# EricLBuehler/mistral.rs

Measured on AMD Instinct MI355X. Metric: decode_tokens_per_sec, higher is better.
Workload: dtype q4_k/q6_k weights x q8_k activations (int8 dot, f32 accumulate: the reference CPU path's arithmetic); 1 GPU; Llama-3-8B GGUF Q4_K_M, TP=1, 512 prefill / 1599 decode, batch 1, paged KV bf16 (block 32); parallelism=tp1

## Files before the change

### include/mrs_hip_ext.h

```cpp
#ifndef MRS_HIP_EXT_H
#define MRS_HIP_EXT_H
#include <stddef.h>
#include <stdint.h>
#ifdef __cplusplus
extern "C" {
#endif

int mrs_decode_gemv_supported(int ggml_type);
int mrs_decode_qkv(const void *wq, const void *wk, const void *wv, int tq, int tk, int tv, int nq, int nk, int nv, int K,
                   const float *h, const float *norm_w, float eps, float *q_out, void *k_cache, void *v_cache,
                   const int64_t *slot_mapping, const int32_t *positions, const float *cos_t, const float *sin_t,
                   int head_dim, int rot_pairs, int num_kv_heads, int block_size, int b, void *stream);
int mrs_decode_gate_up(const void *wg, const void *wu, int type, int n, int K, const float *h, const float *norm_w, float eps,
                       int activation, void *y_out, int y_out_stride, int b, void *stream);
int mrs_decode_proj(const void *w, int type, int n, int K, const void *y_q8_1, int stride_col_y, float *out, int out_stride,
                    int accumulate, int b, void *stream);
int mrs_decode_proj_scaled(const void *w, int type, int n, int K, const void *y_q8_1, int stride_col_y, float *out, int out_stride,
                           float resid_scale, int b, void *stream);
int mrs_vec_add_f32(float *a, const float *b, size_t n, void *stream);
int mrs_decode_norm_proj(const void *w, int type, int n, int K, const float *h, const float *norm_w, float eps, float *out,
                         int out_stride, int b, void *stream);
typedef struct { const void *planes; int type; long long n, k; } mrs_dec_mat;
int mrs_dec_supported(int ggml_type);
size_t mrs_dec_repack_bytes(int ggml_type, long long n, long long k);
int mrs_dec_repack(const void *gguf_blocks, int ggml_type, long long n, long long k, void *planes, void *stream);
int mrs_dec_qkv(const mrs_dec_mat *wq, const mrs_dec_mat *wk, const mrs_dec_mat *wv, const float *h, int ldh, const float *norm_w, float eps,
                float *q_out, void *k_cache, void *v_cache, const int64_t *slot_mapping, const int32_t *positions, const float *cos_t,
                const float *sin_t, int head_dim, int rot_pairs, int num_kv_heads, int block_size, int kv_dtype, int b, void *stream);
int mrs_dec_qkv_neox(const mrs_dec_mat *wq, const mrs_dec_mat *wk, const mrs_dec_mat *wv, const float *h, int ldh, const float *norm_w, float eps,
                     float *q_out, void *k_cache, void *v_cache, const int64_t *slot_mapping, const int32_t *positions, const float *cos_t,
                     const float *sin_t, int head_dim, int rot_pairs, int num_kv_heads, int block_size, int kv_dtype, int b, void *stream);
int mrs_dec_gate_up(const mrs_dec_mat *wg, const mrs_dec_mat *wu, int n, const int32_t *expert_sel, const float *h, int ldh, const float *norm_w,
                    float eps, int activation, float *act_out, int ld_out, int b, void *stream);
int mrs_dec_gate_up_topk(const mrs_dec_mat *wg, const mrs_dec_mat *wu, int n, const int32_t *expert_sel, int topk, const float *h, const float *norm_w, float eps,
                         int activation, float *act_out, int ld_out, void *stream);
int mrs_dec_proj_top2(const mrs_dec_mat *w, int n, const int32_t *expert_sel, const float *x, int ldx, float *out, float resid_scale, const float *acc_scale, void *stream);
int mrs_dec_proj(const mrs_dec_mat *w, int n, const int32_t *expert_sel, const float *x, int ldx, const float *norm_w, float eps, float *out,
                 int ld_out, int mode, float resid_scale, const float *acc_scale, int b, void *stream);
int mrs_dec_proj_argmax(const mrs_dec_mat *w, int n, const float *x, int ldx, const float *norm_w, float eps, float *out, int ld_out, void *amax, void *stream);
size_t mrs_dec_act_image_bytes(int k, int b);
int mrs_dec_attention(float *out_f32, void *img_out, unsigned *ticket, float *part_o, float *part_m, float *part_l, const float *q, const void *k_cache,
                      const void *v_cache, int num_kv_heads, float scale, const uint32_t *block_tables, const uint32_t *context_lens, int block_size,
                      int max_context_len, int num_seqs, int num_heads, int head_size, int max_blocks_per_seq, int q_stride, int kv_block_stride,
                      int kv_head_stride, int kv_dtype, int sliding_window , void *stream);
size_t mrs_dec_proj_img_max_bytes(void);
int mrs_dec_proj_img(const mrs_dec_mat *w, int n, const void *x_img, float *out, int ld_out, int mode, float resid_scale, int b, void *stream);
int mrs_dec_act_image(const float *x, int ldx, const float *norm_w, float eps, int k, int weight_type, int b, void *img_out, void *stream);
int mrs_dec_qkv_img(const mrs_dec_mat *wq, const mrs_dec_mat *wk, const mrs_dec_mat *wv, const void *x_img, float *q_out, void *k_cache, void *v_cache,
                    const int64_t *slot_mapping, const int32_t *positions, const float *cos_t, const float *sin_t, int head_dim, int rot_pairs,
                    int num_kv_heads, int block_size, int kv_dtype, int b, int neox, void *stream);
int mrs_dec_gate_up_img(const mrs_dec_mat *wg, const mrs_dec_mat *wu, int n, const void *x_img, int activation, float *act_out, int ld_out, int b, void *stream);
int mrs_dec_mm_supported(int type, int k, int b);
unsigned long long mrs_dec_mm_launch_count(void);
void mrs_dec_mm_timeline(void *buf);
int mrs_dec_mm_proj(const void *qi, int type, int n, int k, const void *x_img, float *out, int ld_out, int mode, float resid_scale, int b, void *stream);
int mrs_dec_mm_gate_up(const void *qi_gate, const void *qi_up, int type, int n, int k, const void *x_img, int activation, float *act_out, int ld_out, int b, void *stream);
int mrs_dec_mm_qkv(const void *qi_q, int type_q, int nq, const void *qi_k, int type_k, int nk, const void *qi_v, int type_v, int nv, int k, const void *x_img, float *q_out,
                   void *k_cache, void *v_cache, const int64_t *slot_mapping, const int32_t *positions, const float *cos_t, const float *sin_t, int head_dim, int rot_pairs,
                   int num_kv_heads, int block_size, int kv_dtype, int b, void *stream);
int mrs_hqq_gemv(int bits, int dtype, const void *wq, const void *scale, const void *zero, const void *bias, const void *x, int ldx, void *out, int ldo,
                 int N, int K, int b, void *stream);
int mrs_embedding(const void *table, int type, const int32_t *ids, float *out, int K, int tokens, void *stream);
int mrs_sample_advance_embed(int32_t *next_ids, int32_t *tokens_out, int tokens_out_stride, int32_t *step_counter, int32_t *positions, uint32_t *context_lens,
                             int64_t *slot_mapping, const uint32_t *block_tables, int max_blocks, int block_size, void *scratch, const void *table, int type, float *h_next,
                             int K, void *stream);
int mrs_quantize_rows_q8_1(const float *x, void *y, int K, int stride_blocks, int rows, void *stream);
int mrs_sample_greedy_advance(const float *logits, int vocab, int b, int32_t *next_ids, int32_t *tokens_out,
                              int tokens_out_stride, int32_t *step_counter, int32_t *positions, uint32_t *context_lens,
                              int64_t *slot_mapping, const uint32_t *block_tables, int max_blocks, int block_size,
                              void *scratch, void *stream);

int mrs_moe_router_topk(const float *x_normed, const float *gate_w , int tokens, int n_experts, int K, int top_k,
                        int renormalize, int32_t *ids , float *weights ,
                        float *logits_out , void *stream);
int mrs_moe_router_topk_norm(const float *h, const float *norm_w, float eps, const float *gate_w, int tokens, int n_experts, int K, int top_k, int renormalize,
                             int32_t *ids, float *weights, void *stream);
size_t mrs_moe_router_split_scratch_bytes(int tokens, int n_experts);
int mrs_moe_router_topk_norm_split(const float *h, const float *norm_w, float eps, const float *gate_w, int tokens, int n_experts, int K, int top_k, int renormalize,
                                   int32_t *ids, float *weights, void *scratch, void *stream);
int mrs_moe_decode_gate_up(const void *wg, const void *wu, size_t expert_stride_bytes, const int32_t *expert_sel, int type, int n, int K,
                           const float *h, const float *norm_w, float eps, int activation, void *y_out, int y_out_stride, void *stream);
int mrs_moe_decode_down(const void *w, size_t expert_stride_bytes, const int32_t *expert_sel, const float *topk_weight, int type, int n, int K,
                        const void *y_q8_1, int stride_col_y, float *out, void *stream);

// ... 197 lines not shown
```

### mistral.rs_amd/csrc/dec_core2.cuh

```cuda
#pragma once
#include "gguf_blocks.cuh"
#include <type_traits>
#include <utility>

#ifndef MRS_WAVE_SYNC
#define MRS_WAVE_SYNC() __builtin_amdgcn_wave_barrier()
#endif

namespace mrs {
namespace dec2 {

typedef unsigned v4u __attribute__((ext_vector_type(4)));
typedef unsigned v2u __attribute__((ext_vector_type(2)));
#ifndef MRS_DEC2_NT
#define MRS_DEC2_NT 512
#endif
constexpr int NT = MRS_DEC2_NT, NW = NT / 64;

__host__ __device__ inline bool dec_type(int t) { return t == T_Q4_K || t == T_Q5_K || t == T_Q6_K || t == T_Q8_0; }
enum : int { ACT_Q8K = 0, ACT_Q80 = 1 };
__host__ __device__ inline int act_mode_for(int type) { return type == T_Q8_0 ? ACT_Q80 : ACT_Q8K; }

struct Geo { int S, Cs, LPC, TPC, W, R, A; };
__host__ __device__ inline Geo geo_for(int K) {
// ... 397 lines not shown
    const float dwa = half_bits_to_float((uint16_t)(w.dh & 0xffff)), dwb = half_bits_to_float((uint16_t)(w.dh >> 16));
#pragma unroll
    for (int k = 0; k < NCOLS; ++k) {
      const ActQ a = act_quarter(act, col0 + k, qo, c);
      const float2 dx = *(const float2 *)(act.d + ((size_t)(col0 + k) * act.Sp + sb) * act.dw + 2 * c);
      const int isa = dot16(w.q1, a.a1, dot16(w.q0, a.a0, 0)), isb = dot16(w.q3, a.a3, dot16(w.q2, a.a2, 0));
      const float pa = (float)isa * dwa * dx.x, pb = (float)isb * dwb * dx.y;
      float r = pa + pb;
#pragma unroll
      for (int step = 1; step < 4; ++step) {
        const float prev = dppf<0x90>(r);
        const float cand = (prev + pa) + pb;
        r = c == step ? cand : r;
      }
      T[k] = dppf<0xFF>(r);
    }
  }
};

template <int TYPE, int NCOLS, int C0> struct TermCols {
  static __device__ __forceinline__ void run(const typename Tile<TYPE>::Raw &w, int sb, int qo, int c, const Act &act, int col0, float (&T)[NCOLS]) {
    if constexpr (C0 < NCOLS) {
      if constexpr (NCOLS - C0 >= 2) {
        float t2[2];
        Tile<TYPE>::template term<2>(w, sb, qo, c, act, col0 + C0, t2);
        T[C0] = t2[0]; T[C0 + 1] = t2[1];
      } else {
        float t1[1];
        Tile<TYPE>::template term<1>(w, sb, qo, c, act, col0 + C0, t1);
        T[C0] = t1[0];
      }
      if constexpr (C0 + 2 < NCOLS && (C0 & 2) != 0) __builtin_amdgcn_sched_barrier(0);
      TermCols<TYPE, NCOLS, C0 + 2>::run(w, sb, qo, c, act, col0, T);
    }
  }
};

struct Job {
  Mat mat[2];
  int nseg, rgpu;
  int nrows;
  int u0, u1;
  const int32_t *sel;
  int sel_mode;
  int upe;
  int ergs;
  unsigned long long *tl;
};
#define MRS_TL2(jb, i) do { if ((jb).tl && (tid_opaque() & 63) == 0) (jb).tl[((size_t)blockIdx.x * NW + (tid_opaque() >> 6)) * 16 + (i)] = __builtin_amdgcn_s_memrealtime(); } while (0)
__host__ __device__ inline int owner_off(const Geo &) { return 12; }
struct RecMeta { int ts_seg, row0, nvalid; };
struct NoAux {};

template <int TYPE, int NCOLS, bool SEGCOL = false, bool RING2 = false, class Stage, class AuxF, class Epi>
__device__ __forceinline__ void stream(const Job &jb, int K, int ncols_img, int mode, char *smem, int *ctr, bool sbar, Stage stage, AuxF auxf, Epi epi) {
  using TL = Tile<TYPE>;
  using AuxT = decltype(auxf(0));
  constexpr int NS = (NCOLS <= 4 && !RING2) ? TL::NS : (TL::NS > 2 ? 2 : TL::NS);
  const int tid = tid_opaque(), lane = tid & 63, wave = __builtin_amdgcn_readfirstlane(tid >> 6);
  const Geo g = geo_for(K);
  const int Cs = g.Cs;
  constexpr unsigned tileb = tile_bytes(TYPE);
  const int p = (lane >> 2) & 3, c = lane & 3;
  const int nun = jb.u1 - jb.u0 - wave;
  const int myunits = nun > 0 ? (nun + NW - 1) / NW : 0;
  const int tps = jb.rgpu * Cs;
  const int T = myunits * jb.nseg * tps;
  const int tpu = jb.nseg * tps;
  const bool dyn = tpu % NS == 0;
  if (tid == 0) *ctr = jb.u0 + NW;
  if (jb.u0 + wave >= jb.u1) {
    stage(0, wave);
    __syncthreads();
    stage(1, wave);
    if (sbar) __syncthreads();
    stage(2, wave);
    __syncthreads();
    return;
  }
  const __amdgpu_buffer_rsrc_t rs0 = __builtin_amdgcn_make_buffer_rsrc((void *)jb.mat[0].base, (short)0, (int)jb.mat[0].bytes, 0x00020000);
  const bool two = jb.nseg > 1;
  const __amdgpu_buffer_rsrc_t rs1 = __builtin_amdgcn_make_buffer_rsrc((void *)(two ? jb.mat[1].base : jb.mat[0].base), (short)0, (int)(two ? jb.mat[1].bytes : jb.mat[0].bytes), 0x00020000);
  typename TL::Raw ring[NS];
  RecMeta meta[NS];
  AuxT auxv[NS];
  unsigned long long selp = 0ull;
  const bool moe = jb.sel != nullptr;
  if (moe) {
    const int nsl = jb.sel_mode == 2 ? jb.nseg : min(8, (jb.u1 + jb.upe - 1) / jb.upe);
#pragma unroll
    for (int i = 0; i < 8; ++i) if (i < nsl) selp |= (unsigned long long)(unsigned)(__builtin_amdgcn_readfirstlane(jb.sel[i]) & 0xff) << (8 * i);
  }
  auto sel_at = [&](int i) { return (int)((selp >> (8 * (i & 7))) & 0xffull); };
  int lunit = 0, lseg = 0, lleft = 0, lts = 0, lrow0 = 0, lslot_row0 = 0;
  unsigned ltoff = 0, lubase1 = 0;
  auto open_unit = [&](int u) {
    lunit = u; lseg = 0; lts = 0; lleft = tps;
    if (u < jb.u1) {
      int local = u * jb.rgpu, e0 = 0, e1 = 0, sl = 0;
      if (moe) {
        if (jb.sel_mode == 2) { e0 = sel_at(0); e1 = sel_at(1); }
        else { sl = u / jb.upe; e0 = e1 = sel_at(sl); local -= sl * jb.upe * jb.rgpu; }
      }
      ltoff = (unsigned)(e0 * jb.ergs + local) * (unsigned)Cs * tileb;
      lubase1 = (unsigned)(e1 * jb.ergs + local) * (unsigned)Cs * tileb;
      lrow0 = u * jb.rgpu * g.R;
      lslot_row0 = sl * (jb.upe * jb.rgpu * g.R);
    }
  };
  constexpr unsigned DEAD = 0xF0000000u;
  auto issue = [&](typename TL::Raw &slot, RecMeta &m, AuxT &ax) {
    const bool livel = lunit < jb.u1;
    const int lrow = lrow0 - lslot_row0;
    m = RecMeta{livel ? (lts | (lseg << 24)) : -1, lrow0, min(g.R, jb.nrows - lrow)};
    slot = TL::load(lseg == 0 ? rs0 : rs1, livel ? ltoff : DEAD, lane);
    ax = auxf(livel ? lrow0 : 0);
    if (livel) {
      ltoff += tileb;
      if (++lts == Cs) { lts = 0; lrow0 += g.R; }
      if (--lleft == 0) {
        if (lseg + 1 < jb.nseg) { lseg = 1; lleft = tps; ltoff = lubase1; lrow0 -= jb.rgpu * g.R; }
        else if (dyn) {
          int nu = 0;
          if (lane == 0) nu = atomicAdd(ctr, 1);
          open_unit(__builtin_amdgcn_readfirstlane(nu));
        } else open_unit(lunit + NW);
      }
    }
  };
  open_unit(jb.u0 + wave);
  stage(0, wave);
  MRS_TL2(jb, 0);
  __syncthreads();
  issue(ring[0], meta[0], auxv[0]);
  stage(1, wave);
  if (sbar) __syncthreads();
  MRS_TL2(jb, 1);
#pragma unroll
  for (int i = 1; i < NS; ++i) issue(ring[i], meta[i], auxv[i]);
  stage(2, wave);
  MRS_TL2(jb, 2);
  __syncthreads();
  MRS_TL2(jb, 3);
  const Act act = act_view(smem, K, ncols_img, mode);
  const int pCs = p * Cs;
  const int qo_lane = p * act.CQ + c * 64;
  float acc[NCOLS];
#pragma unroll
  for (int k = 0; k < NCOLS; ++k) acc[k] = 0.0f;
  auto compute = [&](int i) {
    const int ts = meta[i].ts_seg & 0xffffff, seg = meta[i].ts_seg >> 24;
    const int sb = pCs + ts;
    const bool live = sb < g.S;
    float Tm[NCOLS];
    TermCols<TYPE, NCOLS, 0>::run(ring[i], sb, qo_lane + ts * 256, c, act, SEGCOL ? seg : 0, Tm);
#pragma unroll
    for (int k = 0; k < NCOLS; ++k) acc[k] = ts == 0 ? (live ? Tm[k] : 0.0f) : (live ? acc[k] + Tm[k] : acc[k]);
    if (ts == Cs - 1) {
      float tot[NCOLS];
#pragma unroll
      for (int k = 0; k < NCOLS; ++k) {
        float u = dppf<0x124>(acc[k]) + acc[k];
        u = dppf<0x124>(u) + acc[k];
        tot[k] = dppf<0x124>(u) + acc[k];
      }
      epi(seg, meta[i].row0, meta[i].nvalid, (meta[i].row0 / g.R) & (jb.rgpu - 1), tot, auxv[i]);
    }
  };
  if (dyn) {
    while (lunit < jb.u1) {
#pragma unroll
      for (int i = 0; i < NS; ++i) { compute(i); issue(ring[i], meta[i], auxv[i]); }
    }
#pragma unroll
    for (int i = 0; i < NS; ++i) compute(i);
  } else {
    const int rest = T > NS ? T - NS : 0;
    const int full = rest / NS;
    for (int ps = 0; ps < full; ++ps) {
#pragma unroll
      for (int i = 0; i < NS; ++i) { compute(i); issue(ring[i], meta[i], auxv[i]); }
    }
    if (rest - full * NS > 0) {
#pragma unroll
      for (int i = 0; i < NS; ++i) { compute(i); issue(ring[i], meta[i], auxv[i]); }
    }
#pragma unroll
    for (int i = 0; i < NS; ++i) if (meta[i].ts_seg >= 0) compute(i);
  }
  MRS_TL2(jb, 14);
}

}
}
```

### mistral.rs_amd/csrc/dec_gemv.cuh

```cuda
#pragma once
#include "dec_core2.cuh"
#include <algorithm>

namespace mrs {
namespace dec {
using namespace mrs::dec2;

enum : int { EPI_STORE = 0, EPI_RESID = 1, EPI_GLU = 2, EPI_QKV = 3, EPI_RESID2 = 4 };

struct GemvArgs {
  Mat m[3];
  int nrows[3];
  int K;
  const float *x; int ldx; const float *norm_w; float eps;
  float *out; int out_stride; float resid_scale;
  int activation;
  float *q_out; void *k_cache, *v_cache; const int64_t *slot_mapping; const int32_t *positions; const float *cos_t, *sin_t;
  int head_dim, rot_pairs, num_kv_heads, block_size, cache_x, kv_f16;
  int hd_shift, bs_shift, x_shift;
  int neox;
  int wg0[4];
  const int32_t *expert_sel;
  const float *acc_scale;
  int slots, slot_out_stride;
  const void *x_img;
  int units[3], rgpu;
  int ubase[3], urem[3], upe;
  unsigned long long *amax;
  unsigned long long *tl;
};
__device__ __forceinline__ unsigned long long pack_max_key(float v, int idx) {
  unsigned u = __float_as_uint(v);
  u = (u & 0x80000000u) ? ~u : (u | 0x80000000u);
  return ((unsigned long long)u << 32) | (unsigned)(0x7fffffff - idx);
}

enum : int { TM_Q4K = 1, TM_Q5K = 2, TM_Q6K = 4, TM_Q80 = 8, TM_ALL = 15 };
__host__ __device__ constexpr int tmask_of(int type) { return type == T_Q4_K ? TM_Q4K : type == T_Q5_K ? TM_Q5K : type == T_Q6_K ? TM_Q6K : type == T_Q8_0 ? TM_Q80 : 0; }
#define MRS_DEC_TYPE_SWITCH(t, ...)                                                              \
  switch (t) {                                                                                   \
  case T_Q4_K: if constexpr ((TMASK & TM_Q4K) != 0) { constexpr int TT = T_Q4_K; __VA_ARGS__ } break; \
  case T_Q5_K: if constexpr ((TMASK & TM_Q5K) != 0) { constexpr int TT = T_Q5_K; __VA_ARGS__ } break; \
  case T_Q6_K: if constexpr ((TMASK & TM_Q6K) != 0) { constexpr int TT = T_Q6_K; __VA_ARGS__ } break; \
  case T_Q8_0: if constexpr ((TMASK & TM_Q80) != 0) { constexpr int TT = T_Q8_0; __VA_ARGS__ } break; \
  default: break;                                                                                \
  }

template <int N> struct AuxV { float a[N], b[N]; };

template <int NCOLS, int EPI, int TMASK, bool RING2>
__device__ __forceinline__ void gemv_phase(const GemvArgs &a, char *smem, float *red, int *ctr, unsigned long long *best) {
  const int tid0 = tid_opaque();
  const int wave = __builtin_amdgcn_readfirstlane(tid0 >> 6), lane = tid0 & 63;
  const int K = a.K;
  const Geo g = geo_for(K);
  const int w1 = a.wg0[1], w2 = a.wg0[2], w3 = a.wg0[3];
  const int un0 = a.units[0], un1 = a.units[1], un2 = a.units[2];
  const int ub0 = a.ubase[0], ub1 = a.ubase[1], ub2 = a.ubase[2], ur0 = a.urem[0], ur1 = a.urem[1], ur2 = a.urem[2];
  const int nr0 = a.nrows[0], nr1 = a.nrows[1], nr2 = a.nrows[2];
  const uint8_t *b0 = a.m[0].base, *b1 = a.m[1].base, *b2 = a.m[2].base;
  const unsigned by0 = a.m[0].bytes, by1 = a.m[1].bytes, by2 = a.m[2].bytes;
  const int ty0 = a.m[0].type, ty1 = a.m[1].type, ty2 = a.m[2].type;
  const int bx = (int)blockIdx.x;
  int mi = 0;
  if constexpr (EPI == EPI_QKV) mi = bx >= w2 ? 2 : (bx >= w1 ? 1 : 0);
  const int wgb = EPI == EPI_QKV ? (mi == 0 ? 0 : (mi == 1 ? w1 : w2)) : 0;
  const int wge = EPI == EPI_QKV ? (mi == 0 ? w1 : (mi == 1 ? w2 : w3)) : (int)gridDim.x;
  const int units = EPI == EPI_QKV ? (mi == 0 ? un0 : (mi == 1 ? un1 : un2)) : un0;
  const int wi = bx - wgb;
  const int ub = EPI == EPI_QKV ? (mi == 0 ? ub0 : (mi == 1 ? ub1 : ub2)) : ub0, ur = EPI == EPI_QKV ? (mi == 0 ? ur0 : (mi == 1 ? ur1 : ur2)) : ur0;
  (void)wge; (void)units;
  Job jb{};
  jb.nseg = (EPI == EPI_GLU || EPI == EPI_RESID2) ? 2 : 1;
  jb.rgpu = a.rgpu;
  jb.mat[0].base = mi == 0 ? b0 : (mi == 1 ? b1 : b2);
  jb.mat[0].bytes = mi == 0 ? by0 : (mi == 1 ? by1 : by2);
  jb.mat[0].type = mi == 0 ? ty0 : (mi == 1 ? ty1 : ty2);
  jb.mat[0].n = 0; jb.mat[0].k = K;
  if constexpr (EPI == EPI_GLU) { jb.mat[1].base = b1; jb.mat[1].bytes = by1; jb.mat[1].type = ty1; jb.mat[1].n = 0; jb.mat[1].k = K; } else jb.mat[1] = jb.mat[0];
  jb.nrows = mi == 0 ? nr0 : (mi == 1 ? nr1 : nr2);
  jb.u0 = wi * ub + min(wi, ur); jb.u1 = jb.u0 + ub + (wi < ur ? 1 : 0);
// ... 40 lines not shown
#pragma unroll
        for (int c = 0; c < NCOLS; ++c) {
          float *o = a.out + (size_t)c * a.out_stride + row0 + rr;
          if constexpr (EPI == EPI_RESID) *o = ax.a[c] * a.resid_scale + sum[c] * ascale;
          else {
            *o = sum[c];
            if constexpr (NCOLS == 1) { if (a.amax) { const unsigned long long key = pack_max_key(sum[c], row0 + rr); *best = key > *best ? key : *best; } }
          }
        }
      }
    };
    MRS_DEC_TYPE_SWITCH(jb.mat[0].type, { stream<TT, NCOLS, false, RING2>(jb, K, NCI, mode, smem, ctr, sbar, stage, auxf, epi); })
  } else if constexpr (EPI == EPI_RESID2) {
    static_assert(EPI != EPI_RESID2 || NCOLS == 1, "one accumulator column; the image has two");
    const float w0 = a.acc_scale[0], w1 = a.acc_scale[1];
    float s0save = 0.0f;
    auto auxf = [&](int row0) {
      AuxV<1> v; v.a[0] = 0.f; v.b[0] = 0.f;
      const int row = row0 + rr;
      v.a[0] = a.out[min(row, jb.nrows - 1)];
      return v;
    };
    auto epi = [&](int seg, int row0, int nvalid, int, const float(&sum)[1], const AuxV<1> &ax) {
      if (seg == 0) {
        s0save = sum[0];
      } else if (own && rr < nvalid) {
        const float h1 = ax.a[0] * a.resid_scale + s0save * w0;
        a.out[row0 + rr] = h1 * 1.0f + sum[0] * w1;
      }
    };
    MRS_DEC_TYPE_SWITCH(jb.mat[0].type, { stream<TT, 1, true, RING2>(jb, K, NCI, mode, smem, ctr, sbar, stage, auxf, epi); })
  } else if constexpr (EPI == EPI_GLU) {
    float gsave[NCOLS];
#pragma unroll
    for (int c = 0; c < NCOLS; ++c) gsave[c] = 0.0f;
    auto auxf = [](int) { return NoAux{}; };
    auto epi = [&](int seg, int row0, int nvalid, int, const float(&sum)[NCOLS], const NoAux &) {
      if (seg == 0) {
#pragma unroll
        for (int c = 0; c < NCOLS; ++c) gsave[c] = sum[c];
      } else if (own && rr < nvalid) {
        const int row = row0 + rr;
        const int slot = a.slots > 1 ? row / a.nrows[0] : 0;
#pragma unroll
        for (int c = 0; c < NCOLS; ++c)
          a.out[(size_t)slot * a.slot_out_stride + (size_t)c * a.out_stride + (row - slot * a.nrows[0])] = (a.activation == 0 ? silu_engine(gsave[c]) : glu_act(gsave[c], a.activation)) * sum[c];
      }
    };
    MRS_DEC_TYPE_SWITCH(jb.mat[0].type, { stream<TT, NCOLS, false, RING2>(jb, K, NCI, mode, smem, ctr, sbar, stage, auxf, epi); })
  } else {
    int posv[NCOLS], slotv[NCOLS];
#pragma unroll
    for (int c = 0; c < NCOLS; ++c) { posv[c] = a.positions[c]; slotv[c] = mi == 0 ? 0 : (int)a.slot_mapping[c]; }
    auto load_aux = [&](int row) {
      AuxV<NCOLS> v;
      const int pair_i = (row & (a.head_dim - 1)) >> 1;
      const bool rot = mi < 2 && pair_i < a.rot_pairs;
      const int pi = min(pair_i, a.rot_pairs - 1);
#pragma unroll
      for (int c = 0; c < NCOLS; ++c) {
        const size_t ti = (size_t)posv[c] * a.rot_pairs + pi;
        const float cs = a.cos_t[ti], sn = a.sin_t[ti];
        v.a[c] = rot ? cs : 1.0f; v.b[c] = rot ? sn : 0.0f;
      }
      return v;
    };
    auto auxf = [&](int row0) {
      if constexpr (AUX_RING) return load_aux(row0 + rr); else return NoAux{};
    };
    float prev[NCOLS];
#pragma unroll
    for (int c = 0; c < NCOLS; ++c) prev[c] = 0.0f;
    auto epi = [&](int, int row0, int nvalid, int rgl, const float(&sum)[NCOLS], const auto &axr) {
      AuxV<NCOLS> ax;
      if constexpr (AUX_RING) ax = axr; else ax = load_aux(row0 + rr);
      const bool single = g.R == 1;
      if (single && (rgl & 1) == 0) {
#pragma unroll
        for (int c = 0; c < NCOLS; ++c) prev[c] = sum[c];
        return;
      }
      const int row = row0 + rr;
      const bool odd = single ? true : (row & 1) != 0;
      const int lr = single ? row - 1 : (row & ~1);
      const int head = lr >> a.hd_shift, dd = lr & (a.head_dim - 1);
      const bool nx = a.neox && mi < 2;
      const int d0 = nx ? dd >> 1 : dd, d1 = nx ? d0 + (a.head_dim >> 1) : dd + 1;
#pragma unroll
      for (int c = 0; c < NCOLS; ++c) {
        const float other = single ? prev[c] : __shfl(sum[c], lane ^ lpr, 64);
        const float xs = odd ? other : sum[c], ys = odd ? sum[c] : other;
        float x, y;
        rope_pair<float>(xs, ys, ax.a[c], ax.b[c], x, y);
        const bool wr0 = single ? own : (own && rr < nvalid && !odd), wr1 = single ? own : (own && rr < nvalid && odd);
        if (wr0 || wr1) {
          if (mi == 0) {
            if (wr0) a.q_out[(size_t)c * a.nrows[0] + head * a.head_dim + d0] = x;
            if (wr1) a.q_out[(size_t)c * a.nrows[0] + head * a.head_dim + d1] = y;
          } else {
            const int slot = slotv[c];
            if (slot >= 0) {
              const unsigned blk = (unsigned)slot >> a.bs_shift, off = (unsigned)slot & (unsigned)(a.block_size - 1);
              uint16_t *kc = (uint16_t *)a.k_cache, *vc = (uint16_t *)a.v_cache;
              const uint16_t xb = a.kv_f16 ? float_to_half_bits(x) : float_to_bf16_bits(x), yb = a.kv_f16 ? float_to_half_bits(y) : float_to_bf16_bits(y);
              if (mi == 1) {
                const int X = a.cache_x;
                const size_t hb = ((size_t)blk * a.num_kv_heads + head) * (size_t)(a.head_dim >> a.x_shift);
                if (wr0) kc[(hb + ((unsigned)d0 >> a.x_shift)) * a.block_size * X + off * X + ((unsigned)d0 & (unsigned)(X - 1))] = xb;
                if (wr1) kc[(hb + ((unsigned)d1 >> a.x_shift)) * a.block_size * X + off * X + ((unsigned)d1 & (unsigned)(X - 1))] = yb;
              } else {
                const size_t o = (((size_t)blk * a.num_kv_heads + head) * a.head_dim + dd) * a.block_size + off;
                if (wr0) vc[o] = xb;
                if (wr1) vc[o + a.block_size] = yb;
              }
            }
          }
        }
      }
    };
    MRS_DEC_TYPE_SWITCH(jb.mat[0].type, { stream<TT, NCOLS, false, RING2>(jb, K, NCI, mode, smem, ctr, sbar, stage, auxf, epi); })
  }
}

template <int NCOLS, int EPI, int TMASK = TM_ALL, bool RING2 = false>
__global__ void __launch_bounds__(NT) dec_gemv_kernel(const GemvArgs a) {
  extern __shared__ __attribute__((aligned(16))) char smem[];
  __shared__ float red[8 * 8];
  __shared__ int ctr;
  if constexpr (EPI == EPI_STORE && NCOLS == 1) {
    __shared__ unsigned long long wbest[NW];
    unsigned long long best = 0ull;
    gemv_phase<NCOLS, EPI, TMASK, RING2>(a, smem, red, &ctr, &best);
    if (a.amax) {
      const int tid = tid_opaque();
#pragma unroll
      for (int m = 32; m > 0; m >>= 1) { const unsigned long long o = __shfl_xor(best, m, 64); best = o > best ? o : best; }
      if ((tid & 63) == 0) wbest[tid >> 6] = best;
      __syncthreads();
      if (tid == 0) {
        unsigned long long b2 = wbest[0];
#pragma unroll
        for (int w = 1; w < NW; ++w) b2 = wbest[w] > b2 ? wbest[w] : b2;
        if (b2) atomicMax(a.amax, b2);
      }
    }
  } else gemv_phase<NCOLS, EPI, TMASK, RING2>(a, smem, red, &ctr, nullptr);
}


template <int NCOLS> int gemv_launch(int epi, int tmask, bool ring2, int grid, size_t lds, const GemvArgs &a, hipStream_t s);

}
}
```

### mistral.rs_amd/csrc/ext_dec.hip

```cpp
#include "dec_attn.cuh"
#include <stdio.h>
#include <stdlib.h>
#include <math.h>
#include <algorithm>
#include "../../include/mistralrs_paged_attn.h"

#include "dec_gemv.cuh"

#ifndef MRS_WAIT_VMCNT0
#define MRS_WAIT_VMCNT0() asm volatile("s_waitcnt vmcnt(0)" ::: "memory")
#endif

namespace mrs {
namespace dec {

__device__ __forceinline__ void st16(uint8_t *p, const uint8_t *b) { *(v4u *)p = *(const v4u *)b; }
__device__ __forceinline__ void k4_scale_min(const uint8_t *sc12, uint8_t *sc, uint8_t *mn) {
#pragma unroll
  for (int g = 0; g < 8; ++g) {
    if (g < 4) { sc[g] = sc12[g] & 63; mn[g] = sc12[g + 4] & 63; }
    else { sc[g] = (sc12[g + 4] & 15) | ((sc12[g - 4] >> 6) << 4); mn[g] = (sc12[g + 4] >> 4) | ((sc12[g] >> 6) << 4); }
  }
}
template <int TYPE>
// ... 239 lines not shown
    if (a.x) a.x += (size_t)c0 * a.ldx;
    if (a.out) a.out += (size_t)c0 * a.out_stride;
    if (a.q_out) a.q_out += (size_t)c0 * a.nrows[0];
    if (a.positions) a.positions += c0;
    if (a.slot_mapping) a.slot_mapping += c0;
    if (a.x_img) a.x_img = (const char *)a.x_img + act_bytes(a.K, c0);
    return a;
  }
  static int run(const GemvArgs &a, int b, hipStream_t s) {
    if (b > 1 && act_bytes(a.K, b) > LDS_IMG_MAX) {
      const int half = b / 2;
      const int rc = run(a, half, s);
      return rc ? rc : run(shift_cols(a, half), b - half, s);
    }
    switch (b) {
    case 1: return go<1>(a, s); case 2: return go<2>(a, s); case 3: return go<3>(a, s); case 4: return go<4>(a, s);
    case 5: return go<5>(a, s); case 6: return go<6>(a, s); case 7: return go<7>(a, s); case 8: return go<8>(a, s);
    default: return -1;
    }
  }
};

}
}

using namespace mrs;
using namespace mrs::dec;

struct mrs_dec_mat_c { const void *planes; int type; long long n, k; };

extern "C" void mrs_dec_timeline(void *buf, int) { g_tl_buf = (unsigned long long *)buf; }
extern "C" int mrs_dec_supported(int ggml_type) { return dec_type(ggml_type) ? 1 : 0; }
extern "C" size_t mrs_dec_repack_bytes(int type, long long n, long long k) {
  if (!dec_type(type) || k <= 0 || k % 256 || n <= 0) return 0;
  return tensor_bytes(type, n, k);
}
extern "C" int mrs_dec_repack(const void *gguf_blocks, int type, long long n, long long k, void *planes, void *stream) {
  if (!mrs_dec_repack_bytes(type, n, k) || !gguf_blocks || !planes) return -1;
  const Geo g = geo_for((int)k);
  const long long nslots = ((n + g.R - 1) / g.R) * g.TPC * 64;
  const dim3 grid((unsigned)((nslots + 255) / 256));
  hipStream_t s = (hipStream_t)stream;
  switch (type) {
  case T_Q4_K: hipLaunchKernelGGL(repack_kernel<T_Q4_K>, grid, dim3(256), 0, s, (const uint8_t *)gguf_blocks, (uint8_t *)planes, n, (int)k, nslots); break;
  case T_Q5_K: hipLaunchKernelGGL(repack_kernel<T_Q5_K>, grid, dim3(256), 0, s, (const uint8_t *)gguf_blocks, (uint8_t *)planes, n, (int)k, nslots); break;
  case T_Q6_K: hipLaunchKernelGGL(repack_kernel<T_Q6_K>, grid, dim3(256), 0, s, (const uint8_t *)gguf_blocks, (uint8_t *)planes, n, (int)k, nslots); break;
  default: hipLaunchKernelGGL(repack_kernel<T_Q8_0>, grid, dim3(256), 0, s, (const uint8_t *)gguf_blocks, (uint8_t *)planes, n, (int)k, nslots); break;
  }
  return 0;
}
static int dec_qkv_impl(const mrs_dec_mat_c *wq, const mrs_dec_mat_c *wk, const mrs_dec_mat_c *wv, const float *h, int ldh, const float *norm_w, float eps,
                        float *q_out, void *k_cache, void *v_cache, const int64_t *slot_mapping, const int32_t *positions, const float *cos_t,
                        const float *sin_t, int head_dim, int rot_pairs, int num_kv_heads, int block_size, int kv_dtype, int b, int neox, void *stream,
                        const void *x_img = nullptr) {
  GemvArgs a{};
  a.neox = neox;
  a.x_img = x_img;
  if (neox && rot_pairs * 2 != head_dim) return -1;
  if (!wq || !wk || !wv || !make_mat(a.m[0], wq->planes, wq->type, wq->n, wq->k) || !make_mat(a.m[1], wk->planes, wk->type, wk->n, wk->k) ||
      !make_mat(a.m[2], wv->planes, wv->type, wv->n, wv->k)) return -1;
  if (wq->k != wk->k || wq->k != wv->k || ((wq->n | wk->n | wv->n | head_dim) & 1)) return -1;
  if (act_mode_for(wq->type) != act_mode_for(wk->type) || act_mode_for(wq->type) != act_mode_for(wv->type)) return -1;
  if (kv_dtype != 0 && kv_dtype != 1) return -1;
  a.nrows[0] = (int)wq->n; a.nrows[1] = (int)wk->n; a.nrows[2] = (int)wv->n; a.K = (int)wq->k;
  a.x = h; a.ldx = ldh; a.norm_w = norm_w; a.eps = eps; a.q_out = q_out; a.k_cache = k_cache; a.v_cache = v_cache; a.slot_mapping = slot_mapping;
  a.positions = positions; a.cos_t = cos_t; a.sin_t = sin_t; a.head_dim = head_dim; a.rot_pairs = rot_pairs; a.num_kv_heads = num_kv_heads;
  a.block_size = block_size; a.cache_x = 8; a.kv_f16 = kv_dtype == 0;
  auto lg2 = [](int v) { int s = 0; while ((1 << s) < v) ++s; return (1 << s) == v ? s : -1; };
  a.hd_shift = lg2(head_dim); a.bs_shift = lg2(block_size); a.x_shift = lg2(a.cache_x);
  if (a.hd_shift < 0 || a.bs_shift < 0 || head_dim < a.cache_x) return -1;
  return Launch<EPI_QKV>::run(a, b, (hipStream_t)stream);
}
extern "C" int mrs_dec_qkv(const mrs_dec_mat_c *wq, const mrs_dec_mat_c *wk, const mrs_dec_mat_c *wv, const float *h, int ldh, const float *norm_w, float eps,
                           float *q_out, void *k_cache, void *v_cache, const int64_t *slot_mapping, const int32_t *positions, const float *cos_t,
                           const float *sin_t, int head_dim, int rot_pairs, int num_kv_heads, int block_size, int kv_dtype, int b, void *stream) {
  return dec_qkv_impl(wq, wk, wv, h, ldh, norm_w, eps, q_out, k_cache, v_cache, slot_mapping, positions, cos_t, sin_t, head_dim, rot_pairs, num_kv_heads, block_size,
                      kv_dtype, b, 0, stream);
}
extern "C" int mrs_dec_qkv_neox(const mrs_dec_mat_c *wq, const mrs_dec_mat_c *wk, const mrs_dec_mat_c *wv, const float *h, int ldh, const float *norm_w, float eps,
                                float *q_out, void *k_cache, void *v_cache, const int64_t *slot_mapping, const int32_t *positions, const float *cos_t,
                                const float *sin_t, int head_dim, int rot_pairs, int num_kv_heads, int block_size, int kv_dtype, int b, void *stream) {
  return dec_qkv_impl(wq, wk, wv, h, ldh, norm_w, eps, q_out, k_cache, v_cache, slot_mapping, positions, cos_t, sin_t, head_dim, rot_pairs, num_kv_heads, block_size,
                      kv_dtype, b, 1, stream);
}

extern "C" int mrs_dec_gate_up(const mrs_dec_mat_c *wg, const mrs_dec_mat_c *wu, int n, const int32_t *expert_sel, const float *h, int ldh, const float *norm_w,
                               float eps, int activation, float *act_out, int ld_out, int b, void *stream) {
  GemvArgs a{};
  if (!wg || !wu || !make_mat(a.m[0], wg->planes, wg->type, wg->n, wg->k) || !make_mat(a.m[1], wu->planes, wu->type, wu->n, wu->k)) return -1;
  if (wg->type != wu->type || wg->n != wu->n || wg->k != wu->k || n <= 0 || wg->n % n || (!expert_sel && wg->n != n) || wg->n / n > 256) return -1;
  a.nrows[0] = a.nrows[1] = n; a.K = (int)wg->k; a.x = h; a.ldx = ldh; a.norm_w = norm_w; a.eps = eps; a.activation = activation;
  a.out = act_out; a.out_stride = ld_out; a.expert_sel = expert_sel;
  return Launch<EPI_GLU>::run(a, b, (hipStream_t)stream);
}

extern "C" int mrs_dec_gate_up_topk(const mrs_dec_mat_c *wg, const mrs_dec_mat_c *wu, int n, const int32_t *expert_sel, int topk, const float *h, const float *norm_w,
                                    float eps, int activation, float *act_out, int ld_out, void *stream) {
  GemvArgs a{};
  if (!wg || !wu || !expert_sel || topk < 1 || topk > 8 || !make_mat(a.m[0], wg->planes, wg->type, wg->n, wg->k) || !make_mat(a.m[1], wu->planes, wu->type, wu->n, wu->k)) return -1;
  if (wg->type != wu->type || wg->n != wu->n || wg->k != wu->k || n <= 0 || wg->n % n || wg->n / n > 256) return -1;
  a.nrows[0] = a.nrows[1] = n; a.K = (int)wg->k; a.x = h; a.ldx = (int)wg->k; a.norm_w = norm_w; a.eps = eps; a.activation = activation;
  a.out = act_out; a.out_stride = ld_out; a.expert_sel = expert_sel; a.slots = topk; a.slot_out_stride = ld_out;
  return Launch<EPI_GLU>::run(a, 1, (hipStream_t)stream);
}

extern "C" int mrs_dec_proj_top2(const mrs_dec_mat_c *w, int n, const int32_t *expert_sel, const float *x, int ldx, float *out, float resid_scale,
                                 const float *acc_scale, void *stream) {
  GemvArgs a{};
  if (!w || !expert_sel || !acc_scale || !make_mat(a.m[0], w->planes, w->type, w->n, w->k) || n <= 0 || w->n % n || w->n / n > 256) return -1;
  a.nrows[0] = n; a.K = (int)w->k; a.x = x; a.ldx = ldx; a.out = out; a.out_stride = n; a.resid_scale = resid_scale; a.acc_scale = acc_scale;
  a.expert_sel = expert_sel;
  return Launch<EPI_RESID2>::go<1>(a, (hipStream_t)stream);
}

extern "C" int mrs_dec_proj(const mrs_dec_mat_c *w, int n, const int32_t *expert_sel, const float *x, int ldx, const float *norm_w, float eps, float *out,
                            int ld_out, int mode, float resid_scale, const float *acc_scale, int b, void *stream) {
  GemvArgs a{};
  if (!w || !make_mat(a.m[0], w->planes, w->type, w->n, w->k) || n <= 0 || w->n % n || (!expert_sel && w->n != n) || w->n / n > 256) return -1;
  a.nrows[0] = n; a.K = (int)w->k; a.x = x; a.ldx = ldx; a.norm_w = norm_w; a.eps = eps; a.out = out; a.out_stride = ld_out;
  a.resid_scale = resid_scale; a.acc_scale = acc_scale; a.expert_sel = expert_sel;
  return mode ? Launch<EPI_RESID>::run(a, b, (hipStream_t)stream) : Launch<EPI_STORE>::run(a, b, (hipStream_t)stream);
}

extern "C" int mrs_dec_proj_argmax(const mrs_dec_mat_c *w, int n, const float *x, int ldx, const float *norm_w, float eps, float *out, int ld_out, void *amax, void *stream) {
  GemvArgs a{};
  if (!w || !amax || !make_mat(a.m[0], w->planes, w->type, w->n, w->k) || n <= 0 || w->n != n) return -1;
  a.nrows[0] = n; a.K = (int)w->k; a.x = x; a.ldx = ldx; a.norm_w = norm_w; a.eps = eps; a.out = out; a.out_stride = ld_out; a.resid_scale = 1.0f;
  a.amax = (unsigned long long *)amax;
  return Launch<EPI_STORE>::run(a, 1, (hipStream_t)stream);
}

extern "C" int mrs_dec_proj_img(const mrs_dec_mat_c *w, int n, const void *x_img, float *out, int ld_out, int mode, float resid_scale, int b, void *stream) {
  GemvArgs a{};
  if (!w || !x_img || !make_mat(a.m[0], w->planes, w->type, w->n, w->k) || n <= 0 || w->n != n) return -1;
  a.nrows[0] = n; a.K = (int)w->k; a.x_img = x_img; a.out = out; a.out_stride = ld_out; a.resid_scale = resid_scale;
  return mode ? Launch<EPI_RESID>::run(a, b, (hipStream_t)stream) : Launch<EPI_STORE>::run(a, b, (hipStream_t)stream);
// ... 69 lines not shown
```

### mistral.rs_amd/csrc/host/runtime.cpp

```cpp
#include <dlfcn.h>
#include <hip/hip_runtime.h>

#include <cstdarg>
#include <cstdlib>
#include <cstdio>
#include <cmath>
#include <cstring>
#include <algorithm>
#include <initializer_list>
#include <memory>
#include <string>
#include <vector>

#include "../../../include/mistralrs_core.h"
#include "../../../include/mistralrs_paged_attn.h"
#include "../../../include/mistralrs_quant.h"
#include "../../../include/mrs_hip_ext.h"

namespace mrs_host {

static thread_local std::string g_last_error;
int fail(const char *fmt, ...) {
  char buf[512];
  va_list ap;
// ... 335 lines not shown
        }
        continue;
      }
      const QTensor *g = bl.gate_proj->get_qtensor(), *u = bl.up_proj->get_qtensor(), *dn = bl.down_proj->get_qtensor();
      if (mrs_decode_gate_up(g->data, u->data, g->dtype, ff, d, ws.h, bl.post_attention_layernorm, cfg.rms_eps, 0, ws.y_b, stride_f, b, s))
        return fail("mrs_decode_gate_up refused");
      if (mrs_decode_proj_scaled(dn->data, dn->dtype, d, ff, ws.y_b, stride_f, ws.h, d, rs, b, s) || all_reduce(ws.h, (size_t)b * d, s)) return fail("down_proj failed: %s", g_last_error.c_str());
    }
    const QTensor *lm = lm_head->get_qtensor();
    if (mrs_decode_norm_proj(lm->data, lm->dtype, cfg.vocab_size, d, ws.h, ln_f, cfg.rms_eps, bufs.logits, cfg.vocab_size, b, s))
      return fail("mrs_decode_norm_proj refused");
    return 0;
  }

  bool engine_ok() const {
    if (cfg.use_fused != 2 || cfg.head_dim != 128 || cfg.block_size != 32 || (cfg.head_dim & 1)) return false;
    if (!cfg.rope_interleaved && cfg.rot_dim != cfg.head_dim) return false;
    const int g = cfg.num_heads / cfg.num_kv_heads;
    if (g != 1 && g != 2 && g != 4 && g != 8) return false;
    if (!dlm_head.planes) return false;
    for (const Block &bl : blocks) {
      if (!bl.dq.planes || !bl.dk.planes || !bl.dv.planes || !bl.dout.planes) return false;
      if ((bl.dq.type == Q8_0) != (bl.dk.type == Q8_0) || (bl.dq.type == Q8_0) != (bl.dv.type == Q8_0)) return false;
      if (cfg.num_experts > 0) {
        if (!bl.dgate_exps.planes || !bl.dup_exps.planes || !bl.ddown_exps.planes || bl.dgate_exps.type != bl.dup_exps.type) return false;
      } else if (!bl.dgate.planes || !bl.dup.planes || !bl.ddown.planes || bl.dgate.type != bl.dup.type) return false;
    }
    return true;
  }
  int forward_engine(int b, hipStream_t s, bool chained = false) const {
    const float rs = 1.0f / (float)std::max(1, (int)cfg.world_size);
    const int d = cfg.hidden_size, hd = cfg.head_dim, nq = cfg.num_heads * hd, ff = cfg.intermediate_size, kvd = cfg.kv_f16 ? 0 : 1;
    const int bs = cfg.block_size, kvh = cfg.num_kv_heads;
    const int eff_max = std::min(cfg.max_blocks_per_seq * bs, cfg.max_context_len);
    if (chained && b != 1) return fail("chained decode step: batch 1 only");
    if (!chained && wte->embedding_forward_raw(bufs.input_ids, b, ws.h, s)) return -1;
    const bool imgb = b >= 2 && b <= 8;
    auto image = [&](const float *x, int ldx, const float *nw, int k, int wtype) { return mrs_dec_act_image(x, ldx, nw, cfg.rms_eps, k, wtype, b, ws.act_img, s); };
    constexpr int mm_min_b = 3;
    const bool mmb = imgb && b >= mm_min_b;
    auto qi_of = [](const std::unique_ptr<GgufMatMul> &l) -> const void * { return l && l->get_qtensor() ? l->get_qtensor()->qi : nullptr; };
    auto mm_ok = [&](const void *qi, int type, int k) { return mmb && qi && mrs_dec_mm_supported(type, k, b); };
    for (const Block &bl : blocks) {
      if (imgb && cfg.rope_interleaved && mm_ok(qi_of(bl.q_proj), bl.dq.type, d) && mm_ok(qi_of(bl.k_proj), bl.dk.type, d) && mm_ok(qi_of(bl.v_proj), bl.dv.type, d)) {
        if (image(ws.h, d, bl.input_layernorm, d, bl.dq.type) ||
            mrs_dec_mm_qkv(qi_of(bl.q_proj), bl.dq.type, (int)bl.dq.n, qi_of(bl.k_proj), bl.dk.type, (int)bl.dk.n, qi_of(bl.v_proj), bl.dv.type, (int)bl.dv.n, d, ws.act_img, ws.q,
                           bl.key_cache, bl.value_cache, bufs.slot_mapping, bufs.positions, bufs.cos_table, bufs.sin_table, hd, cfg.rot_dim / 2, kvh, bs, kvd, b, s))
          return fail("mrs_dec_mm_qkv refused the layer");
      } else if (imgb) {
        if (image(ws.h, d, bl.input_layernorm, d, bl.dq.type) ||
            mrs_dec_qkv_img(&bl.dq, &bl.dk, &bl.dv, ws.act_img, ws.q, bl.key_cache, bl.value_cache, bufs.slot_mapping, bufs.positions, bufs.cos_table, bufs.sin_table, hd,
                            cfg.rot_dim / 2, kvh, bs, kvd, b, cfg.rope_interleaved ? 0 : 1, s))
          return fail("mrs_dec_qkv_img refused the layer");
      } else if ((cfg.rope_interleaved ? mrs_dec_qkv : mrs_dec_qkv_neox)(&bl.dq, &bl.dk, &bl.dv, ws.h, d, bl.input_layernorm, cfg.rms_eps, ws.q, bl.key_cache, bl.value_cache,
                                                                  bufs.slot_mapping, bufs.positions, bufs.cos_table, bufs.sin_table, hd, cfg.rot_dim / 2, kvh, bs, kvd, b, s))
        return fail("mrs_dec_qkv refused the layer");
      const bool want_img = bl.dout.type != 8 && (cfg.num_heads / kvh) % 2 == 0 && mrs_dec_act_image_bytes(nq, b) <= mrs_dec_proj_img_max_bytes();
      const int rc2 = mrs_dec_attention(want_img ? nullptr : ws.attn, want_img ? ws.attn_img : nullptr, ws.attn_ticket, (float *)ws.attn_ws, ws.max_logits, ws.exp_sums, ws.q,
                                        bl.key_cache, bl.value_cache, kvh, 1.0f / sqrtf((float)hd), bufs.block_tables, bufs.context_lens, bs, eff_max, b, cfg.num_heads, hd,
                                        cfg.max_blocks_per_seq, nq, kvh * hd * bs, hd * bs, kvd, cfg.sliding_window, s);
      if (rc2 < 0) return fail("mrs_dec_attention refused the shape");
      const int prc = rc2 == 1 ? (mm_ok(qi_of(bl.o_proj), bl.dout.type, nq) ? mrs_dec_mm_proj(qi_of(bl.o_proj), bl.dout.type, d, nq, ws.attn_img, ws.h, d, 1, rs, b, s)
                                                                              : mrs_dec_proj_img(&bl.dout, d, ws.attn_img, ws.h, d, 1, rs, b, s))
                               : mrs_dec_proj(&bl.dout, d, nullptr, ws.attn, nq, nullptr, 0.f, ws.h, d, 1, rs, nullptr, b, s);
      if (prc || all_reduce(ws.h, (size_t)b * d, s)) return fail("o_proj failed (%d): %s", prc, g_last_error.c_str());
      if (cfg.num_experts > 0) {
        const int E = cfg.num_experts, tk = cfg.num_experts_per_tok;
        const int rrc = mrs_moe_router_topk_norm_split(ws.h, bl.post_attention_layernorm, cfg.rms_eps, bl.router, b, E, d, tk, 1, ws.moe_ids, ws.moe_w, ws.moe_router_scratch, s);
        if (rrc == -3) {
          mrs_rms_norm_f32(ws.h, bl.post_attention_layernorm, ws.xn, b, d, cfg.rms_eps, (int64_t)(intptr_t)s);
          if (mrs_moe_router_topk(ws.xn, bl.router, b, E, d, tk, 1, ws.moe_ids, ws.moe_w, nullptr, s)) return fail("moe router refused (experts %d, top-k %d)", E, tk);
        } else if (rrc) return fail("moe router refused (experts %d, top-k %d)", E, tk);
        for (int t = 0; t < b; ++t) {
          float *ht = ws.h + (size_t)t * d;
          const int grc = mrs_dec_gate_up_topk(&bl.dgate_exps, &bl.dup_exps, ff, ws.moe_ids + t * tk, tk, ht, bl.post_attention_layernorm, cfg.rms_eps, 0, ws.moe_act, ff, s);
          if (grc != 0 && grc != -3) return fail("moe gate/up refused (%d)", grc);
          for (int sl = 0; grc == -3 && sl < tk; ++sl)
            if (mrs_dec_gate_up(&bl.dgate_exps, &bl.dup_exps, ff, ws.moe_ids + t * tk + sl, ht, d, bl.post_attention_layernorm, cfg.rms_eps, 0,
                                ws.moe_act + (size_t)sl * ff, ff, 1, s))
              return fail("moe gate/up refused");
          if (tk == 2 && grc == 0 && mrs_dec_proj_top2(&bl.ddown_exps, d, ws.moe_ids + t * tk, ws.moe_act, ff, ht, rs, ws.moe_w + t * tk, s) == 0) continue;
          for (int sl = 0; sl < tk; ++sl)
            if (mrs_dec_proj(&bl.ddown_exps, d, ws.moe_ids + t * tk + sl, ws.moe_act + (size_t)sl * ff, ff, nullptr, 0.f, ht, d, 1, sl == 0 ? rs : 1.0f, ws.moe_w + t * tk + sl, 1, s))
              return fail("moe down refused");
        }
        if (all_reduce(ws.h, (size_t)b * d, s)) return fail("moe all-reduce failed: %s", g_last_error.c_str());
        continue;
      }
      if (imgb) {
        const bool mmg = mm_ok(qi_of(bl.gate_proj), bl.dgate.type, d) && qi_of(bl.up_proj);
        if (image(ws.h, d, bl.post_attention_layernorm, d, bl.dgate.type) ||
            (mmg ? mrs_dec_mm_gate_up(qi_of(bl.gate_proj), qi_of(bl.up_proj), bl.dgate.type, ff, d, ws.act_img, 0, ws.act, ff, b, s)
                 : mrs_dec_gate_up_img(&bl.dgate, &bl.dup, ff, ws.act_img, 0, ws.act, ff, b, s)))
          return fail("mrs_dec_gate_up_img refused");
      } else if (mrs_dec_gate_up(&bl.dgate, &bl.dup, ff, nullptr, ws.h, d, bl.post_attention_layernorm, cfg.rms_eps, 0, ws.act, ff, b, s)) return fail("mrs_dec_gate_up refused");
      const int drc = imgb ? (image(ws.act, ff, nullptr, ff, bl.ddown.type) ||
                              (mm_ok(qi_of(bl.down_proj), bl.ddown.type, ff) ? mrs_dec_mm_proj(qi_of(bl.down_proj), bl.ddown.type, d, ff, ws.act_img, ws.h, d, 1, rs, b, s)
                                                                               : mrs_dec_proj_img(&bl.ddown, d, ws.act_img, ws.h, d, 1, rs, b, s)))
                                                    : mrs_dec_proj(&bl.ddown, d, nullptr, ws.act, ff, nullptr, 0.f, ws.h, d, 1, rs, nullptr, b, s);
      if (drc || all_reduce(ws.h, (size_t)b * d, s)) return fail("down_proj failed: %s", g_last_error.c_str());
    }
    const int lrc = chained ? mrs_dec_proj_argmax(&dlm_head, cfg.vocab_size, ws.h, d, ln_f, cfg.rms_eps, bufs.logits, cfg.vocab_size, ws.sample_scratch, s)
                    : imgb ? (image(ws.h, d, ln_f, d, dlm_head.type) ||
                              (mm_ok(qi_of(lm_head), dlm_head.type, d) ? mrs_dec_mm_proj(qi_of(lm_head), dlm_head.type, cfg.vocab_size, d, ws.act_img, bufs.logits, cfg.vocab_size, 0, 1.0f, b, s)
                                                                        : mrs_dec_proj_img(&dlm_head, cfg.vocab_size, ws.act_img, bufs.logits, cfg.vocab_size, 0, 1.0f, b, s)))
                           : mrs_dec_proj(&dlm_head, cfg.vocab_size, nullptr, ws.h, d, ln_f, cfg.rms_eps, bufs.logits, cfg.vocab_size, 0, 1.0f, nullptr, b, s);
// ... 616 lines not shown
```

Before: 534.6 tokens/s.

## Warm L2 with upcoming KV cache pages during the fused QKV GEMV

Adds a side hook to the streaming GEMV core. In the batch-1 QKV kernel this hook issues loads of paged K/V cache lines that the following attention kernel will read, and the loaded values are pinned in registers so the compiler keeps the loads. The goal is to overlap KV cache fetches with weight streaming, so attention finds its data already in cache. In exchange it adds extra memory traffic and register pressure to the QKV kernel, and it only applies when the shape is 8 KV heads, head_dim 128 and block 32.

```diff
diff --git a/include/mrs_hip_ext.h b/include/mrs_hip_ext.h
--- a/include/mrs_hip_ext.h
+++ b/include/mrs_hip_ext.h
@@ -30,6 +30,10 @@
 int mrs_dec_qkv_neox(const mrs_dec_mat *wq, const mrs_dec_mat *wk, const mrs_dec_mat *wv, const float *h, int ldh, const float *norm_w, float eps,
                      float *q_out, void *k_cache, void *v_cache, const int64_t *slot_mapping, const int32_t *positions, const float *cos_t,
                      const float *sin_t, int head_dim, int rot_pairs, int num_kv_heads, int block_size, int kv_dtype, int b, void *stream);
+int mrs_dec_qkv_kv_ahead(const mrs_dec_mat *wq, const mrs_dec_mat *wk, const mrs_dec_mat *wv, const float *h, int ldh, const float *norm_w, float eps,
+                         float *q_out, void *k_cache, void *v_cache, const int64_t *slot_mapping, const int32_t *positions, const float *cos_t,
+                         const float *sin_t, int head_dim, int rot_pairs, int num_kv_heads, int block_size, int kv_dtype, int b, int neox,
+                         const uint32_t *block_tables, const uint32_t *context_lens, int max_blocks_per_seq, int kv_block_stride, int kv_head_stride, void *stream);
 int mrs_dec_gate_up(const mrs_dec_mat *wg, const mrs_dec_mat *wu, int n, const int32_t *expert_sel, const float *h, int ldh, const float *norm_w,
                     float eps, int activation, float *act_out, int ld_out, int b, void *stream);
 int mrs_dec_gate_up_topk(const mrs_dec_mat *wg, const mrs_dec_mat *wu, int n, const int32_t *expert_sel, int topk, const float *h, const float *norm_w, float eps,
diff --git a/mistral.rs_amd/csrc/dec_core2.cuh b/mistral.rs_amd/csrc/dec_core2.cuh
--- a/mistral.rs_amd/csrc/dec_core2.cuh
+++ b/mistral.rs_amd/csrc/dec_core2.cuh
@@ -473,8 +473,9 @@
 struct RecMeta { int ts_seg, row0, nvalid; };
 struct NoAux {};
 
-template <int TYPE, int NCOLS, bool SEGCOL = false, bool RING2 = false, class Stage, class AuxF, class Epi>
-__device__ __forceinline__ void stream(const Job &jb, int K, int ncols_img, int mode, char *smem, int *ctr, bool sbar, Stage stage, AuxF auxf, Epi epi) {
+struct NoSide { __device__ __forceinline__ void operator()() const {} };
+template <int TYPE, int NCOLS, bool SEGCOL = false, bool RING2 = false, class Stage, class AuxF, class Epi, class Side = NoSide>
+__device__ __forceinline__ void stream(const Job &jb, int K, int ncols_img, int mode, char *smem, int *ctr, bool sbar, Stage stage, AuxF auxf, Epi epi, Side side = Side{}) {
   using TL = Tile<TYPE>;
   using AuxT = decltype(auxf(0));
   constexpr int NS = (NCOLS <= 4 && !RING2) ? TL::NS : (TL::NS > 2 ? 2 : TL::NS);
@@ -495,6 +496,7 @@
     __syncthreads();
     stage(1, wave);
     if (sbar) __syncthreads();
+    side();
     stage(2, wave);
     __syncthreads();
     return;
@@ -593,6 +595,7 @@
 #pragma unroll
       for (int i = 0; i < NS; ++i) { compute(i); issue(ring[i], meta[i], auxv[i]); }
     }
+    side();
 #pragma unroll
     for (int i = 0; i < NS; ++i) compute(i);
   } else {
@@ -606,6 +609,7 @@
 #pragma unroll
       for (int i = 0; i < NS; ++i) { compute(i); issue(ring[i], meta[i], auxv[i]); }
     }
+    side();
 #pragma unroll
     for (int i = 0; i < NS; ++i) if (meta[i].ts_seg >= 0) compute(i);
   }
diff --git a/mistral.rs_amd/csrc/dec_gemv.cuh b/mistral.rs_amd/csrc/dec_gemv.cuh
--- a/mistral.rs_amd/csrc/dec_gemv.cuh
+++ b/mistral.rs_amd/csrc/dec_gemv.cuh
@@ -1,6 +1,14 @@
 #pragma once
 #include "dec_core2.cuh"
 #include <algorithm>
+
+#ifndef MRS_KEEP_VGPR
+#ifdef __AMDGCN__
+#define MRS_KEEP_VGPR(x) asm volatile("" ::"v"(x))
+#else
+#define MRS_KEEP_VGPR(x) ((void)(x))
+#endif
+#endif
 
 namespace mrs {
 namespace dec {
@@ -27,6 +35,8 @@
   int units[3], rgpu;
   int ubase[3], urem[3], upe;
   unsigned long long *amax;
+  const uint32_t *pf_bt, *pf_ctx;
+  int pf_max_blocks, pf_block_stride, pf_head_stride;
   unsigned long long *tl;
 };
 __device__ __forceinline__ unsigned long long pack_max_key(float v, int idx) {
@@ -173,6 +183,37 @@
     int posv[NCOLS], slotv[NCOLS];
 #pragma unroll
     for (int c = 0; c < NCOLS; ++c) { posv[c] = a.positions[c]; slotv[c] = mi == 0 ? 0 : (int)a.slot_mapping[c]; }
+    constexpr int KVPF = NCOLS == 1 ? 4 : 0;
+    const uint16_t *pfp[KVPF > 0 ? KVPF : 1];
+    if constexpr (KVPF > 0) {
+      const bool on = a.pf_bt != nullptr;
+      const uint32_t *btp = on ? a.pf_bt : (const uint32_t *)a.positions, *ctxp = on ? a.pf_ctx : (const uint32_t *)a.positions;
+      const int kvh = bx & 7, nslots = ((w3 - kvh + 7) >> 3) * NW, slot0 = (bx >> 3) * NW + wave;
+      unsigned page[KVPF];
+#pragma unroll
+      for (int i = 0; i < KVPF; ++i) page[i] = btp[on ? min((slot0 + i * nslots) >> 4, a.pf_max_blocks - 1) : 0];
+      const int nld = on ? (((int)ctxp[0] + 31) >> 5) * 16 : 0;
+#pragma unroll
+      for (int i = 0; i < KVPF; ++i) {
+        const int it = slot0 + i * nslots;
+        const uint16_t *base = (it & 8) ? (const uint16_t *)a.v_cache : (const uint16_t *)a.k_cache;
+        const size_t off = (size_t)page[i] * (size_t)a.pf_block_stride + (size_t)kvh * (size_t)a.pf_head_stride + (size_t)(it & 7) * 512;
+        pfp[i] = it < nld ? base + off : (const uint16_t *)a.k_cache;
+      }
+    }
+    v4u pfv[KVPF > 0 ? KVPF : 1];
+    auto kv_ahead = [&]() {
+      if constexpr (KVPF > 0) {
+#pragma unroll
+        for (int i = 0; i < KVPF; ++i) pfv[i] = *(const v4u *)(pfp[i] + lane * 8);
+      }
+    };
+    auto kv_ahead_done = [&]() {
+      if constexpr (KVPF > 0) {
+#pragma unroll
+        for (int i = 0; i < KVPF; ++i) MRS_KEEP_VGPR(pfv[i]);
+      }
+    };
     auto load_aux = [&](int row) {
       AuxV<NCOLS> v;
       const int pair_i = (row & (a.head_dim - 1)) >> 1;
@@ -239,7 +280,8 @@
         }
       }
     };
-    MRS_DEC_TYPE_SWITCH(jb.mat[0].type, { stream<TT, NCOLS, false, RING2>(jb, K, NCI, mode, smem, ctr, sbar, stage, auxf, epi); })
+    MRS_DEC_TYPE_SWITCH(jb.mat[0].type, { stream<TT, NCOLS, false, RING2>(jb, K, NCI, mode, smem, ctr, sbar, stage, auxf, epi, kv_ahead); })
+    kv_ahead_done();
   }
 }
 
diff --git a/mistral.rs_amd/csrc/ext_dec.hip b/mistral.rs_amd/csrc/ext_dec.hip
--- a/mistral.rs_amd/csrc/ext_dec.hip
+++ b/mistral.rs_amd/csrc/ext_dec.hip
@@ -315,9 +315,14 @@
 static int dec_qkv_impl(const mrs_dec_mat_c *wq, const mrs_dec_mat_c *wk, const mrs_dec_mat_c *wv, const float *h, int ldh, const float *norm_w, float eps,
                         float *q_out, void *k_cache, void *v_cache, const int64_t *slot_mapping, const int32_t *positions, const float *cos_t,
                         const float *sin_t, int head_dim, int rot_pairs, int num_kv_heads, int block_size, int kv_dtype, int b, int neox, void *stream,
-                        const void *x_img = nullptr) {
+                        const void *x_img = nullptr, const uint32_t *pf_bt = nullptr, const uint32_t *pf_ctx = nullptr, int pf_max_blocks = 0, int pf_block_stride = 0,
+                        int pf_head_stride = 0) {
   GemvArgs a{};
   a.neox = neox;
+  if (pf_bt && pf_ctx && b == 1 && num_kv_heads == 8 && head_dim == 128 && block_size == 32 && pf_max_blocks >= 1 && pf_head_stride >= head_dim * block_size &&
+      pf_block_stride >= num_kv_heads * pf_head_stride) {
+    a.pf_bt = pf_bt; a.pf_ctx = pf_ctx; a.pf_max_blocks = pf_max_blocks; a.pf_block_stride = pf_block_stride; a.pf_head_stride = pf_head_stride;
+  }
   a.x_img = x_img;
   if (neox && rot_pairs * 2 != head_dim) return -1;
   if (!wq || !wk || !wv || !make_mat(a.m[0], wq->planes, wq->type, wq->n, wq->k) || !make_mat(a.m[1], wk->planes, wk->type, wk->n, wk->k) ||
@@ -345,6 +350,15 @@
                                 const float *sin_t, int head_dim, int rot_pairs, int num_kv_heads, int block_size, int kv_dtype, int b, void *stream) {
   return dec_qkv_impl(wq, wk, wv, h, ldh, norm_w, eps, q_out, k_cache, v_cache, slot_mapping, positions, cos_t, sin_t, head_dim, rot_pairs, num_kv_heads, block_size,
                       kv_dtype, b, 1, stream);
+}
+
+extern "C" int mrs_dec_qkv_kv_ahead(const mrs_dec_mat_c *wq, const mrs_dec_mat_c *wk, const mrs_dec_mat_c *wv, const float *h, int ldh, const float *norm_w, float eps,
+                                    float *q_out, void *k_cache, void *v_cache, const int64_t *slot_mapping, const int32_t *positions, const float *cos_t,
+                                    const float *sin_t, int head_dim, int rot_pairs, int num_kv_heads, int block_size, int kv_dtype, int b, int neox,
+                                    const uint32_t *block_tables, const uint32_t *context_lens, int max_blocks_per_seq, int kv_block_stride, int kv_head_stride,
+                                    void *stream) {
+  return dec_qkv_impl(wq, wk, wv, h, ldh, norm_w, eps, q_out, k_cache, v_cache, slot_mapping, positions, cos_t, sin_t, head_dim, rot_pairs, num_kv_heads, block_size,
+                      kv_dtype, b, neox ? 1 : 0, stream, nullptr, block_tables, context_lens, max_blocks_per_seq, kv_block_stride, kv_head_stride);
 }
 
 extern "C" int mrs_dec_gate_up(const mrs_dec_mat_c *wg, const mrs_dec_mat_c *wu, int n, const int32_t *expert_sel, const float *h, int ldh, const float *norm_w,
diff --git a/mistral.rs_amd/csrc/host/runtime.cpp b/mistral.rs_amd/csrc/host/runtime.cpp
--- a/mistral.rs_amd/csrc/host/runtime.cpp
+++ b/mistral.rs_amd/csrc/host/runtime.cpp
@@ -411,6 +411,11 @@
             mrs_dec_qkv_img(&bl.dq, &bl.dk, &bl.dv, ws.act_img, ws.q, bl.key_cache, bl.value_cache, bufs.slot_mapping, bufs.positions, bufs.cos_table, bufs.sin_table, hd,
                             cfg.rot_dim / 2, kvh, bs, kvd, b, cfg.rope_interleaved ? 0 : 1, s))
           return fail("mrs_dec_qkv_img refused the layer");
+      } else if (b == 1) {
+        if (mrs_dec_qkv_kv_ahead(&bl.dq, &bl.dk, &bl.dv, ws.h, d, bl.input_layernorm, cfg.rms_eps, ws.q, bl.key_cache, bl.value_cache, bufs.slot_mapping, bufs.positions,
+                                 bufs.cos_table, bufs.sin_table, hd, cfg.rot_dim / 2, kvh, bs, kvd, b, cfg.rope_interleaved ? 0 : 1, bufs.block_tables, bufs.context_lens,
+                                 cfg.max_blocks_per_seq, kvh * hd * bs, hd * bs, s))
+          return fail("mrs_dec_qkv_kv_ahead refused the layer");
       } else if ((cfg.rope_interleaved ? mrs_dec_qkv : mrs_dec_qkv_neox)(&bl.dq, &bl.dk, &bl.dv, ws.h, d, bl.input_layernorm, cfg.rms_eps, ws.q, bl.key_cache, bl.value_cache,
                                                                   bufs.slot_mapping, bufs.positions, bufs.cos_table, bufs.sin_table, hd, cfg.rot_dim / 2, kvh, bs, kvd, b, s))
         return fail("mrs_dec_qkv refused the layer");
```

New measurement: 527.3 tokens/s (median of 2 runs). 1.4% lower.
